# Algy/fast-slic

Hardware: NVIDIA H100
Metric: megapixels/sec (10 iters, K=1600) (higher is better)
Workload: dtype u8/u16 integer

## Files before the change

### fast_slic_b200/csrc/cca.cuh

```cuda
#pragma once
#include "common.cuh"

#define CCA_BLOCK 1024
#define CCA_HIST 2052

struct CcaParams {
    int H, W, N;
    int K;
    int thres;
    int nblk;
    int heap_in_smem;
    int which;
};

__device__ __forceinline__ bool cca_skip_image(const CcaParams& cp, const struct CcaCounters* ct);

struct CcaCounters {
    int ncomp;
    int ncand;
    int nkept;
    int sel_mode;
    int keep_thres;
    int need_sim;
    int dbg_ops;
    int dbg_t;
};

__device__ __forceinline__ bool cca_skip_image(const CcaParams& cp, const CcaCounters* ct) {
    return cp.which >= 0 && (ct->need_sim != 0) != (cp.which != 0);
}

__device__ __forceinline__ int ccl_find(const int* par, int x) {
    int p = par[x];
    while (p != x) {
        x = p;
        p = par[x];
    }
    return x;
}

__device__ __forceinline__ void ccl_union(int* par, int a, int b) {
    a = ccl_find(par, a);
    b = ccl_find(par, b);
    while (a != b) {
        if (a < b) {
            int t = a;
            a = b;
            b = t;
        }
        const int old = atomicMin(&par[a], b);
        if (old == a) break;
        a = ccl_find(par, old);
        b = ccl_find(par, b);
    }
}

#define CCL_T 32

#define CCL_TW 4
__global__ void __launch_bounds__(32 * CCL_TW) k_ccl_tile(CcaParams cp, const uint16_t* __restrict__ labels,
                                                          int* __restrict__ par_all, uint32_t* __restrict__ area_all,
                                                          int tiles_x, int tiles_y, long ntiles_total) {
    __shared__ int s_par_all[CCL_TW][CCL_T * CCL_T];
    const int lane = threadIdx.x & 31, warp = threadIdx.x >> 5;
    const long tile = (long)blockIdx.x * CCL_TW + warp;
    if (tile >= ntiles_total) return;
    int* s_par = s_par_all[warp];
    const int per_img = tiles_x * tiles_y;
    const int b = (int)(tile / per_img);
    const int tl = (int)(tile - (long)b * per_img);
    const int tyb = tl / tiles_x, txb = tl - tyb * tiles_x;
    const int j = txb * CCL_T + lane;
    const bool colok = j < cp.W;
    const int nrows = min(CCL_T, cp.H - tyb * CCL_T);
    const uint16_t* lab = labels + (size_t)b * cp.N + (size_t)(tyb * CCL_T) * cp.W + j;
    constexpr int CCL_G = 8;
    uint32_t v[CCL_G], nv[CCL_G];
#pragma unroll
    for (int k = 0; k < CCL_G; k++) {
        v[k] = (colok && k < nrows) ? (uint32_t)lab[(size_t)k * cp.W] : (0x10000u + (uint32_t)(k * CCL_T + lane));
    }
    uint32_t up_v = 0xffffffffu, up_left = 0xffffffffu;
    int up_root = 0;
#pragma unroll 1
    for (int ty0 = 0; ty0 < CCL_T; ty0 += CCL_G) {
#pragma unroll
        for (int k = 0; k < CCL_G; k++) {
            const int ty = ty0 + CCL_G + k;
            nv[k] = (colok && ty < nrows) ? (uint32_t)lab[(size_t)ty * cp.W] : (0x10000u + (uint32_t)((ty & (CCL_T - 1)) * CCL_T + lane));
        }
#pragma unroll
        for (int k = 0; k < CCL_G; k++) {
            const int ty = ty0 + k;
            const uint32_t cur = v[k];
            const uint32_t left = __shfl_up_sync(FSLIC_FULL, cur, 1);
            const bool start = (lane == 0) || (cur != left);
            const unsigned m = __ballot_sync(FSLIC_FULL, start);
            const int sl = 31 - __clz(m & (0xffffffffu >> (31 - lane)));
            const unsigned above = (lane == 31) ? 0u : (m >> (lane + 1));
            const int end = above ? (lane + __ffs(above) - 1) : 31;
            const bool conn = (ty > 0) && (up_v == cur);
            const bool need = conn && ((lane == 0) || (left != cur) || (up_left != up_v));
            unsigned cand = 0xffffffffu;
            if (need) cand = (unsigned)ccl_find(s_par, up_root);
            unsigned pm = cand;
#pragma unroll
            for (int o = 1; o < 32; o <<= 1) {
                const unsigned y = __shfl_up_sync(FSLIC_FULL, pm, o);
                if (lane - o >= sl) pm = min(pm, y);
            }
            const unsigned rmin = __shfl_sync(FSLIC_FULL, pm, end);
            const unsigned own = (unsigned)(ty * CCL_T + sl);
            const int root = (int)(rmin < own ? rmin : own);
            if (need && cand != (unsigned)root) ccl_union(s_par, (int)cand, root);
            s_par[ty * CCL_T + lane] = root;
            __syncwarp();
            up_left = left;
            up_v = cur;
            up_root = root;
        }
#pragma unroll
        for (int k = 0; k < CCL_G; k++) v[k] = nv[k];
    }
    if (!colok) return;
    int* pout = par_all + (size_t)b * cp.N + (size_t)(tyb * CCL_T) * cp.W + j;
    uint32_t* aout = area_all + (size_t)b * cp.N + (size_t)(tyb * CCL_T) * cp.W + j;
#pragma unroll 4
    for (int ty = 0; ty < nrows; ty++) {
        const int rt = ccl_find(s_par, ty * CCL_T + lane);
        const int ri = tyb * CCL_T + (rt >> 5), rj = txb * CCL_T + (rt & 31);
        pout[(size_t)ty * cp.W] = ri * cp.W + rj;
        aout[(size_t)ty * cp.W] = 0;
    }
}

__global__ void __launch_bounds__(256) k_ccl_seams(CcaParams cp, const uint16_t* __restrict__ labels,
                                                   int* __restrict__ par_all) {
    const int b = blockIdx.y;
    const int W = cp.W, H = cp.H;
    const int sv = (W - 1) / CCL_T, sh = (H - 1) / CCL_T;
    const int nV = sv * H, nH = sh * W;
    const uint16_t* lab = labels + (size_t)b * cp.N;
    int* par = par_all + (size_t)b * cp.N;
    for (int t = blockIdx.x * blockDim.x + threadIdx.x; t < nV + nH; t += gridDim.x * blockDim.x) {
        if (t < nV) {
            const int i = t / sv, j = (t - i * sv + 1) * CCL_T;
            const int p = i * W + j;
            if (lab[p - 1] == lab[p]) ccl_union(par, p - 1, p);
        } else {
            const int u = t - nV;
            const int r = u / W, j = u - r * W;
            const int i = (r + 1) * CCL_T;
            const int p = i * W + j;
            const uint16_t v = lab[p], up = lab[p - W];
            if (up == v) {
                bool need = (j % CCL_T == 0) || (lab[p - 1] != v);
                if (!need) need = lab[p - W - 1] != up;
                if (need) ccl_union(par, p - W, p);
            }
        }
    }
}

__global__ void __launch_bounds__(256) k_ccl_flatten(CcaParams cp, const uint16_t* __restrict__ labels,
                                                     int* __restrict__ par_all, uint32_t* __restrict__ area_all,
                                                     int* __restrict__ blkcnt, int* __restrict__ rootbuf_all,
                                                     int* __restrict__ predbuf_all,
                                                     unsigned long long* __restrict__ chunkinfo_all) {
    __shared__ int s_chunk[32];
    const int b = blockIdx.y;
    const int lane = threadIdx.x & 31, w = threadIdx.x >> 5;
    const uint16_t* lab = labels + (size_t)b * cp.N;
    int* par = par_all + (size_t)b * cp.N;
    int p[4], sl[4], root[4];
    unsigned m[4], rmask[4];
    bool ok[4], start[4], col0[4];
    int jcol = (blockIdx.x * CCA_BLOCK + w * 128 + lane) % cp.W;
#pragma unroll
    for (int r = 0; r < 4; r++) {
        p[r] = blockIdx.x * CCA_BLOCK + (w * 4 + r) * 32 + lane;
        ok[r] = p[r] < cp.N;
        const uint32_t v = ok[r] ? lab[p[r]] : 0x10000u;
        const uint32_t left = __shfl_up_sync(FSLIC_FULL, v, 1);
        const int j = jcol;
        col0[r] = j == 0;
        jcol += 32;
        if (jcol >= cp.W) jcol = (cp.W >= 32) ? (jcol - cp.W) : (jcol % cp.W);
        start[r] = (lane == 0) || (j == 0) || (v != left);
        m[r] = __ballot_sync(FSLIC_FULL, start[r]);
        sl[r] = 31 - __clz(m[r] & (0xffffffffu >> (31 - lane)));
    }
    {
        int q[4];
#pragma unroll
        for (int r = 0; r < 4; r++) {
            root[r] = p[r];
            q[r] = (ok[r] && start[r]) ? par[p[r]] : p[r];
        }
        for (;;) {
            bool mv[4], any = false;
#pragma unroll
            for (int r = 0; r < 4; r++) {
                mv[r] = q[r] != root[r];
                root[r] = q[r];
                any |= mv[r];
            }
            if (!any) break;
#pragma unroll
            for (int r = 0; r < 4; r++)
                if (mv[r]) q[r] = par[root[r]];
        }
    }
    int pred[4], findq[4];
    int prev_last = 0;
#pragma unroll
    for (int r = 0; r < 4; r++) {
        const int rt = __shfl_sync(FSLIC_FULL, root[r], sl[r]);
        const int left_rt = __shfl_up_sync(FSLIC_FULL, rt, 1);
        const int last_rt = __shfl_sync(FSLIC_FULL, rt, 31);
        bool isroot = false;
        pred[r] = -1;
        findq[r] = -1;
        if (ok[r]) {
            par[p[r]] = rt;
            if (start[r]) {
                const unsigned above = (lane == 31) ? 0u : (m[r] >> (lane + 1));
                int len = above ? (__ffs(above)) : (32 - lane);
                if (p[r] + len > cp.N) len = cp.N - p[r];
                atomicAdd(&area_all[(size_t)b * cp.N + rt], (uint32_t)len);
                isroot = (rt == p[r]);
                if (isroot && p[r] > 0) {
                    if (col0[r]) findq[r] = p[r] - cp.W;
                    else if (lane > 0) pred[r] = left_rt;
                    else if (r > 0) pred[r] = prev_last;
                    else findq[r] = p[r] - 1;
                }
            }
        }
        prev_last = last_rt;
        rmask[r] = __ballot_sync(FSLIC_FULL, isroot);
        if (lane == 0) s_chunk[w * 4 + r] = __popc(rmask[r]);
    }
#pragma unroll
    for (int r = 0; r < 4; r++)
        if (findq[r] >= 0) pred[r] = ccl_find(par, findq[r]);
    __syncthreads();
    const int mine = s_chunk[lane];
    int incl = mine;
#pragma unroll
    for (int o = 1; o < 32; o <<= 1) {
        const int y = __shfl_up_sync(FSLIC_FULL, incl, o);
        if (lane >= o) incl += y;
    }
    int* rootbuf = rootbuf_all + (size_t)b * cp.N + (size_t)blockIdx.x * CCA_BLOCK;
    int* predbuf = predbuf_all + (size_t)b * cp.N + (size_t)blockIdx.x * CCA_BLOCK;
#pragma unroll
    for (int r = 0; r < 4; r++) {
        const int base = __shfl_sync(FSLIC_FULL, incl - mine, w * 4 + r);
        if ((rmask[r] >> lane) & 1u) {
            const int e = base + __popc(rmask[r] & ((1u << lane) - 1u));
            rootbuf[e] = p[r];
            predbuf[e] = pred[r];
        }
        if (lane == 0)
            chunkinfo_all[((size_t)b * cp.nblk + blockIdx.x) * (CCA_BLOCK / 32) + w * 4 + r] =
                ((unsigned long long)(unsigned)base << 32) | rmask[r];
    }
    if (threadIdx.x == 31) blkcnt[(size_t)b * cp.nblk + blockIdx.x] = incl;
}

__global__ void __launch_bounds__(1024) k_scan_blocks(const int* __restrict__ cnt_all, int* __restrict__ off_all,
                                                      int stride_per_image, int n_static,
                                                      const int* __restrict__ n_dev_base, int n_dev_stride_ints,
                                                      int n_div, int* __restrict__ total_base,
                                                      int total_stride_ints,
                                                      const CcaCounters* __restrict__ skip_counters, int which) {
    __shared__ int s_warp[32];
    __shared__ int s_carry;
    const int b = blockIdx.x;
    if (skip_counters && which >= 0 && (skip_counters[b].need_sim != 0) != (which != 0)) return;
    const int tid = threadIdx.x;
    const int* cnt = cnt_all + (size_t)b * stride_per_image;
    int* off = off_all + (size_t)b * stride_per_image;
    int n = n_static;
    if (n_dev_base) n = (n_dev_base[(size_t)b * n_dev_stride_ints] + n_div - 1) / n_div;
    if (tid == 0) s_carry = 0;
    __syncthreads();
    for (int base = 0; base < n; base += 1024) {
        const int c = base + tid;
        const int v = (c < n) ? cnt[c] : 0;
        int x = v;
#pragma unroll
        for (int o = 1; o < 32; o <<= 1) {
            int y = __shfl_up_sync(FSLIC_FULL, x, o);
            if ((tid & 31) >= o) x += y;
        }
        if ((tid & 31) == 31) s_warp[tid >> 5] = x;
        __syncthreads();
        if (tid < 32) {
            int w = s_warp[tid];
#pragma unroll
            for (int o = 1; o < 32; o <<= 1) {
                int y = __shfl_up_sync(FSLIC_FULL, w, o);
                if (tid >= o) w += y;
            }
            s_warp[tid] = w;
        }
        __syncthreads();
        const int woff = (tid >> 5) ? s_warp[(tid >> 5) - 1] : 0;
        const int excl = s_carry + woff + x - v;
        if (c < n) off[c] = excl;
        __syncthreads();
        if (tid == 1023) s_carry = excl + v;
        __syncthreads();
    }
    if (tid == 0) total_base[(size_t)b * total_stride_ints] = s_carry;
}

#define CCA_NUMBER_GRID 16
__global__ void __launch_bounds__(CCA_BLOCK) k_ccl_number(CcaParams cp, const int* __restrict__ rootbuf_all,
                                                          const uint32_t* __restrict__ aux_all,
                                                          const int* __restrict__ blkcnt,
                                                          const int* __restrict__ blkoff,
                                                          uint32_t* __restrict__ carea_all,
                                                          CcaCounters* __restrict__ counters,
                                                          unsigned int* __restrict__ ahist_all) {
    __shared__ int s_cand;
    __shared__ unsigned int s_hot[CCA_BLOCK / 32][32];
    const int b = blockIdx.y;
    const int lane = threadIdx.x & 31, warp = threadIdx.x >> 5;
    s_hot[warp][lane] = 0;
    if (threadIdx.x == 0) s_cand = 0;
    __syncthreads();
    const uint32_t* aux = aux_all + (size_t)b * cp.N;
    int ncand = 0;
    constexpr int NU = 8;
    const int wpi = gridDim.x * (CCA_BLOCK / 32);
    const int NB = (cp.nblk + wpi - 1) / wpi;
    for (int blk0 = (blockIdx.x * (CCA_BLOCK / 32) + warp) * NB; blk0 < cp.nblk; blk0 += wpi * NB) {
        for (int sub = 0; sub < NB; sub += 32) {
            const int myblk = blk0 + sub + lane;
            const bool have = (sub + lane < NB) && (myblk < cp.nblk);
            const int mycnt = have ? blkcnt[(size_t)b * cp.nblk + myblk] : 0;
            const int myoff = have ? blkoff[(size_t)b * cp.nblk + myblk] : 0;
            int incl = mycnt;
#pragma unroll
            for (int o = 1; o < 32; o <<= 1) {
                const int y = __shfl_up_sync(FSLIC_FULL, incl, o);
                if (lane >= o) incl += y;
            }
            const int total = __shfl_sync(FSLIC_FULL, incl, 31);
            const int nb_here = min(32, NB - sub);
            for (int r0 = 0; r0 < total; r0 += 32 * NU) {
                int pp[NU], cc[NU];
                uint32_t aa[NU];
#pragma unroll
                for (int u = 0; u < NU; u++) {
                    const int r = r0 + 32 * u + lane;
                    int bi = 0;
                    for (int q = 0; q < nb_here - 1; q++) bi += (r >= __shfl_sync(FSLIC_FULL, incl, q));
                    const int bincl = __shfl_sync(FSLIC_FULL, incl, bi), bcnt = __shfl_sync(FSLIC_FULL, mycnt, bi);
                    const int boff = __shfl_sync(FSLIC_FULL, myoff, bi);
                    const int t = r - (bincl - bcnt);
                    pp[u] = -1;
                    if (r < total) {
                        pp[u] = rootbuf_all[(size_t)b * cp.N + (size_t)(blk0 + sub + bi) * CCA_BLOCK + t];
                        cc[u] = boff + t;
                    }
                }
#pragma unroll
                for (int u = 0; u < NU; u++) aa[u] = pp[u] != -1 ? aux[pp[u]] : 0u;
#pragma unroll
                for (int u = 0; u < NU; u++) {
                    uint32_t bin = 0xffffffffu;
                    if (pp[u] != -1) {
                        carea_all[(size_t)b * cp.N + cc[u]] = aa[u];
                        if ((int)aa[u] >= cp.thres) bin = aa[u] < 2048u ? aa[u] : 2048u;
                    }
                    const unsigned peers = __match_any_sync(FSLIC_FULL, bin);
                    if (bin != 0xffffffffu && lane == __ffs(peers) - 1) {
                        const unsigned n = __popc(peers);
                        ncand += (int)n;
                        if (bin < 32u) s_hot[warp][bin] += n;
                        else atomicAdd(&ahist_all[(size_t)b * CCA_HIST + bin], n);
                    }
                    __syncwarp();
                }
            }
        }
    }
    ncand = __reduce_add_sync(FSLIC_FULL, ncand);
    if (lane == 0 && ncand) atomicAdd(&s_cand, ncand);
    __syncthreads();
    if (threadIdx.x == 0 && s_cand) atomicAdd(&counters[b].ncand, s_cand);
    if (threadIdx.x < 32) {
        unsigned int tot = 0;
        for (int w = 0; w < CCA_BLOCK / 32; w++) tot += s_hot[w][threadIdx.x];
        if (tot) atomicAdd(&ahist_all[(size_t)b * CCA_HIST + threadIdx.x], tot);
    }
}

__global__ void __launch_bounds__(1024) k_cca_threshold(CcaParams cp, const uint32_t* __restrict__ carea_all,
                                                        CcaCounters* __restrict__ counters,
                                                        const unsigned int* __restrict__ ahist_all) {
    __shared__ unsigned int s_hist[2048];
    __shared__ int s_warp[32];
    __shared__ unsigned int s_prefix, s_rank, s_found_bin, s_found_cnt;
    const int b = blockIdx.x;
    const int tid = threadIdx.x, lane = tid & 31, warp = tid >> 5;
    CcaCounters* ct = &counters[b];
    const int ncomp = ct->ncomp, ncand = ct->ncand;
    if (ncand <= cp.K) {
        if (tid == 0) {
            ct->keep_thres = cp.thres;
            ct->sel_mode = 0;
            ct->need_sim = 0;
        }
        return;
    }
    const uint32_t* area = carea_all + (size_t)b * cp.N;
    if (tid == 0) {
// ... 470 lines not shown
    const int b = blockIdx.y;
    if (cca_skip_image(cp, &counters[b])) return;
    const int ncomp = counters[b].ncomp;
    const int sel_mode = counters[b].sel_mode, keep_thres = counters[b].keep_thres;
    const int tid = threadIdx.x, lane = tid & 31, warp = tid >> 5;
    const uint32_t* carea = carea_all + (size_t)b * cp.N;
    for (int blk0 = blockIdx.x * CCA_KEPT_U; blk0 * CCA_BLOCK < ncomp; blk0 += gridDim.x * CCA_KEPT_U) {
        uint32_t a[CCA_KEPT_U];
        int off[CCA_KEPT_U];
#pragma unroll
        for (int u = 0; u < CCA_KEPT_U; u++) {
            const int c = (blk0 + u) * CCA_BLOCK + tid;
            a[u] = (c < ncomp) ? carea[c] : 0u;
            off[u] = ((blk0 + u) * CCA_BLOCK < ncomp) ? blkoff[(size_t)b * cp.nblk + blk0 + u] : 0;
        }
        unsigned m[CCA_KEPT_U];
        bool kept[CCA_KEPT_U];
        __syncthreads();
#pragma unroll
        for (int u = 0; u < CCA_KEPT_U; u++) {
            const int c = (blk0 + u) * CCA_BLOCK + tid;
            kept[u] = (c < ncomp) && cca_is_kept(a[u], sel_mode, keep_thres);
            m[u] = __ballot_sync(FSLIC_FULL, kept[u]);
            if (lane == 0) s_warp[u][warp] = __popc(m[u]);
        }
        __syncthreads();
        if (warp < CCA_KEPT_U) {
            const int w = s_warp[warp][lane];
            int x = w;
#pragma unroll
            for (int o = 1; o < 32; o <<= 1) {
                const int y = __shfl_up_sync(FSLIC_FULL, x, o);
                if (lane >= o) x += y;
            }
            s_warp[warp][lane] = x - w;
        }
        __syncthreads();
#pragma unroll
        for (int u = 0; u < CCA_KEPT_U; u++) {
            const int c = (blk0 + u) * CCA_BLOCK + tid;
            if (c < ncomp) {
                uint16_t v = (c == 0) ? 0 : 0xFFFF;
                if (kept[u]) v = (uint16_t)(off[u] + s_warp[u][warp] + __popc(m[u] & ((1u << lane) - 1)));
                cnew_all[(size_t)b * cp.N + c] = v;
            }
        }
    }
}

#define CCA_TAIL_WARPS 8

__device__ __forceinline__ int cca_comp_of_root(const unsigned long long* chunkinfo, const int* blkoff, int x,
                                                int& slot) {
    const unsigned long long ci = chunkinfo[x >> 5];
    const int local = (int)(ci >> 32) + __popc((uint32_t)ci & ((1u << (x & 31)) - 1u));
    slot = (x >> 10) * CCA_BLOCK + local;
    return blkoff[x >> 10] + local;
}

__device__ __forceinline__ unsigned cca_ld_label(const uint16_t* p) {
    unsigned short v;
    asm volatile("ld.relaxed.gpu.global.u16 %0, [%1];" : "=h"(v) : "l"(p));
    return v;
}
__device__ __forceinline__ void cca_st_label(uint16_t* p, unsigned v) {
    asm volatile("st.relaxed.gpu.global.u16 [%0], %1;" ::"l"(p), "h"((unsigned short)v));
}

__global__ void __launch_bounds__(32 * CCA_TAIL_WARPS) k_cca_absorb(CcaParams cp, const int* __restrict__ rootbuf_all,
                                                                   const int* __restrict__ predbuf_all,
                                                                   const unsigned long long* __restrict__ chunkinfo_all,
                                                                   const int* __restrict__ blkoff_all,
                                                                   const CcaCounters* __restrict__ counters,
                                                                   uint16_t* cnew_all, uint16_t* __restrict__ final_all,
                                                                   int nsplit) {
    const int b = blockIdx.y;
    if (cca_skip_image(cp, &counters[b])) return;
    const int lane = threadIdx.x & 31, gw = blockIdx.x * CCA_TAIL_WARPS + (threadIdx.x >> 5);
    const int blk = gw / nsplit, part = gw - blk * nsplit;
    if (blk >= cp.nblk) return;
    const int* blkoff = blkoff_all + (size_t)b * cp.nblk;
    const int off = blkoff[blk];
    const int n = ((blk + 1 < cp.nblk) ? blkoff[blk + 1] : counters[b].ncomp) - off;
    const int* roots = rootbuf_all + (size_t)b * cp.N + (size_t)blk * CCA_BLOCK;
    const int* preds = predbuf_all + (size_t)b * cp.N;
    const unsigned long long* chunkinfo = chunkinfo_all + (size_t)b * cp.nblk * (CCA_BLOCK / 32);
    uint16_t* cnew = cnew_all + (size_t)b * cp.N;
    uint16_t* fin = final_all + (size_t)b * cp.N;
    constexpr int NU = 8;
    for (int t0 = 32 * part; t0 < n; t0 += 32 * nsplit * NU) {
        int rt[NU], x[NU];
        unsigned lab[NU];
#pragma unroll
        for (int u = 0; u < NU; u++) {
            const int t = t0 + 32 * nsplit * u + lane;
            rt[u] = -1;
            x[u] = 0;
            lab[u] = 0;
            if (t < n) {
                rt[u] = roots[t];
                x[u] = preds[(size_t)blk * CCA_BLOCK + t];
                lab[u] = cnew[off + t];
            }
        }
        int cx[NU], slot[NU];
        unsigned pl[NU];
        bool act[NU];
#pragma unroll
        for (int u = 0; u < NU; u++) {
            act[u] = rt[u] >= 0 && lab[u] == 0xFFFFu;
            pl[u] = 0;
            if (act[u]) cx[u] = cca_comp_of_root(chunkinfo, blkoff, x[u], slot[u]);
        }
        for (;;) {
            bool any = false;
#pragma unroll
            for (int u = 0; u < NU; u++) pl[u] = act[u] ? cca_ld_label(cnew + cx[u]) : pl[u];
#pragma unroll
            for (int u = 0; u < NU; u++) {
                if (act[u] && pl[u] != 0xFFFFu) {
                    act[u] = false;
                    lab[u] = pl[u];
                    cca_st_label(cnew + off + t0 + 32 * nsplit * u + lane, pl[u]);
                }
                any |= act[u];
            }
            if (!any) break;
            int q[NU];
#pragma unroll
            for (int u = 0; u < NU; u++) q[u] = act[u] ? preds[slot[u]] : 0;
#pragma unroll
            for (int u = 0; u < NU; u++)
                if (act[u]) cx[u] = cca_comp_of_root(chunkinfo, blkoff, q[u], slot[u]);
        }
#pragma unroll
        for (int u = 0; u < NU; u++) {
            if (rt[u] < 0) continue;
            fin[rt[u]] = (uint16_t)lab[u];
        }
    }
}

__global__ void __launch_bounds__(256) k_cca_output(CcaParams cp, const int* __restrict__ par_all,
                                                    const uint16_t* __restrict__ final_all,
                                                    uint16_t* __restrict__ out_all,
                                                    const CcaCounters* __restrict__ counters) {
    const int b = blockIdx.y;
    if (cca_skip_image(cp, &counters[b])) return;
    const int* par = par_all + (size_t)b * cp.N;
    const uint16_t* fin = final_all + (size_t)b * cp.N;
    uint16_t* out = out_all + (size_t)b * cp.N;
    if ((cp.N & 7) == 0 && (reinterpret_cast<uintptr_t>(out_all) & 15) == 0 && (reinterpret_cast<uintptr_t>(par_all) & 15) == 0) {
        for (int t = blockIdx.x * blockDim.x + threadIdx.x; t < cp.N / 8; t += gridDim.x * blockDim.x) {
            const int4 r0 = reinterpret_cast<const int4*>(par)[2 * t], r1 = reinterpret_cast<const int4*>(par)[2 * t + 1];
            const uint32_t a0 = fin[r0.x];
            uint32_t a1 = a0, a2, a3, a4, a5, a6, a7;
            if (r0.y != r0.x) a1 = fin[r0.y];
            a2 = a1; if (r0.z != r0.y) a2 = fin[r0.z];
            a3 = a2; if (r0.w != r0.z) a3 = fin[r0.w];
            a4 = a3; if (r1.x != r0.w) a4 = fin[r1.x];
            a5 = a4; if (r1.y != r1.x) a5 = fin[r1.y];
            a6 = a5; if (r1.z != r1.y) a6 = fin[r1.z];
            a7 = a6; if (r1.w != r1.z) a7 = fin[r1.w];
            reinterpret_cast<uint4*>(out)[t] = make_uint4(a0 | (a1 << 16), a2 | (a3 << 16), a4 | (a5 << 16), a6 | (a7 << 16));
        }
        return;
    }
    for (int p = blockIdx.x * blockDim.x + threadIdx.x; p < cp.N; p += gridDim.x * blockDim.x) out[p] = fin[par[p]];
}
```

### fast_slic_b200/csrc/cca_stage.cu

```cuda
#include <stdlib.h>
#include <algorithm>
#include <type_traits>

#include "capi_common.h"
#include "cca.cuh"
#include "cca_stage.h"

struct CcaScratch {
    int* par;
    uint32_t* aux;
    uint32_t* carea;
    uint16_t* cnew;
    uint16_t* fin;
    int* rootbuf;
    int* predbuf;
    unsigned long long* chunkinfo;
    int* blkcnt;
    int* blkoff;
    int* kblkoff;
    CcaCounters* counters;
    unsigned int* ahist;
    unsigned long long* heap;
    size_t total;
};

static CcaScratch cca_layout(void* base, int N, int images, int slot) {
    CcaScratch x;
    Carve c(base);
    auto take = [&](auto*& p, size_t per_image) {
        using T = std::remove_reference_t<decltype(*p)>;
        p = c.take<T>((size_t)images * per_image * sizeof(T));
        if (p) p += (size_t)slot * per_image;
    };
    const size_t n = (size_t)N, nblk = (size_t)ceil_div(N, CCA_BLOCK);
    take(x.par, n);
    take(x.aux, n);
    take(x.carea, n);
    x.cnew = c.take<uint16_t>((size_t)images * n * 2 * sizeof(uint16_t));
    x.fin = x.cnew ? x.cnew + ((size_t)images + slot) * n : nullptr;
    if (x.cnew) x.cnew += (size_t)slot * n;
    take(x.rootbuf, n);
    take(x.predbuf, n);
    take(x.chunkinfo, nblk * (CCA_BLOCK / 32));
    take(x.blkcnt, nblk);
    take(x.blkoff, nblk);
    take(x.kblkoff, nblk);
    take(x.counters, 1);
    take(x.ahist, CCA_HIST);
    take(x.heap, CCA_HEAP_K);
    x.total = c.total;
    return x;
}

static CcaScratch cca_window(const CcaStage& s, int slot) { return cca_layout(s.scratch, s.N, s.batch, slot); }

cudaError_t cca_stage_create(CcaStage& s, int H, int W, int max_batch, size_t device_bytes, int num_sms, int max_smem_optin) {
    s.H = H; s.W = W; s.N = H * W; s.num_sms = num_sms; s.max_smem_optin = max_smem_optin;
    const size_t per_img = (size_t)s.N * 26 + 4096;
    size_t cap = 12ull << 30;
    if (device_bytes && device_bytes / 8 < cap) cap = device_bytes / 8;
    size_t bc = cap / per_img;
    if (bc < 1) bc = 1;
    if (bc > (size_t)max_batch) bc = max_batch;
    if (const char* e = getenv("FSLIC_CCA_BATCH")) {
        const long v = atol(e);
        if (v >= 1 && (size_t)v < bc) bc = (size_t)v;
    }
    s.batch = (int)bc;
    cudaError_t e = cudaMalloc(&s.scratch, cca_layout(nullptr, s.N, s.batch, 0).total);
    if (e == cudaSuccess) e = cudaMemset(cca_window(s, 0).counters, 0, bc * sizeof(CcaCounters));
    if (e == cudaSuccess) e = cudaMallocHost(reinterpret_cast<void**>(&s.h_counters), 64 * sizeof(CcaCounters));
    for (auto& ev : s.ev)
        if (e == cudaSuccess) e = cudaEventCreate(&ev);
    for (CcaLane& l : s.lanes) {
        if (e == cudaSuccess) e = cudaStreamCreateWithFlags(&l.side, cudaStreamNonBlocking);
        for (cudaEvent_t* ev : {&l.fork, &l.join, &l.tail})
            if (e == cudaSuccess) e = cudaEventCreateWithFlags(ev, cudaEventDisableTiming);
    }
    if (e == cudaSuccess)
        e = cudaFuncSetAttribute(k_cca_select, cudaFuncAttributeMaxDynamicSharedMemorySize, max_smem_optin - 4 * 1024);
    if (e == cudaSuccess)
        e = cudaFuncSetAttribute(k_debug_heap_select, cudaFuncAttributeMaxDynamicSharedMemorySize, max_smem_optin - 4 * 1024);
    return e;
}

void cca_stage_destroy(CcaStage& s) {
    if (s.scratch) cudaFree(s.scratch);
    if (s.h_counters) cudaFreeHost(s.h_counters);
    for (cudaEvent_t e : s.ev)
        if (e) cudaEventDestroy(e);
    for (const CcaLane& l : s.lanes) {
        if (l.side) cudaStreamDestroy(l.side);
        for (cudaEvent_t e : {l.fork, l.join, l.tail})
            if (e) cudaEventDestroy(e);
    }
}

static int number_grid(int nblk, int nb) {
    return nb >= 8 ? CCA_NUMBER_GRID : std::min(std::max(ceil_div(nblk, 32), CCA_NUMBER_GRID), 64);
}

static int cca_label(const CcaStage& s, const CcaScratch& x, const CcaParams& cp, const uint16_t* in, int nb, bool timed,
                     cudaStream_t st) {
    if (timed) CK(cudaEventRecord(s.ev[0], st));
    CK(cudaMemsetAsync(x.counters, 0, sizeof(CcaCounters) * nb, st));
    CK(cudaMemsetAsync(x.ahist, 0, sizeof(unsigned int) * CCA_HIST * nb, st));
    dim3 g(cp.nblk, nb);
    {
        const int ttx = ceil_div(s.W, CCL_T), tty = ceil_div(s.H, CCL_T);
        const long ntt = (long)ttx * tty * nb;
        k_ccl_tile<<<(int)((ntt + CCL_TW - 1) / CCL_TW), 32 * CCL_TW, 0, st>>>(cp, in, x.par, x.aux, ttx, tty, ntt);
    }
    {
        const int seam_px = ((s.W - 1) / CCL_T) * s.H + ((s.H - 1) / CCL_T) * s.W;
        if (seam_px > 0) {
            dim3 gs(ceil_div(seam_px, 256), nb);
            k_ccl_seams<<<gs, 256, 0, st>>>(cp, in, x.par);
        }
    }
    if (timed) CK(cudaEventRecord(s.ev[1], st));
    k_ccl_flatten<<<g, 256, 0, st>>>(cp, in, x.par, x.aux, x.blkcnt, x.rootbuf, x.predbuf, x.chunkinfo);
    k_scan_blocks<<<nb, 1024, 0, st>>>(x.blkcnt, x.blkoff, cp.nblk, cp.nblk, nullptr, 0, 1,
                                       &x.counters[0].ncomp, (int)(sizeof(CcaCounters) / sizeof(int)), nullptr, -1);
    k_ccl_number<<<dim3(number_grid(cp.nblk, nb), nb), CCA_BLOCK, 0, st>>>(cp, x.rootbuf, x.aux, x.blkcnt, x.blkoff,
                                                                            x.carea, x.counters, x.ahist);
    if (timed) CK(cudaEventRecord(s.ev[2], st));
    k_cca_threshold<<<nb, 1024, 0, st>>>(cp, x.carea, x.counters, x.ahist);
    if (timed) CK(cudaEventRecord(s.ev[3], st));
    return FSLIC_OK;
}

static void cca_finish(const CcaStage& s, const CcaScratch& x, const CcaParams& cp, int which, uint16_t* out, int nb,
                       bool timed, cudaStream_t ts) {
    CcaParams cq = cp;
    cq.which = which;
    const dim3 gk(std::min(cp.nblk, std::max(CCA_KEPT_GRID, 256 / nb)), nb);
    k_kept_count<<<gk, CCA_BLOCK, 0, ts>>>(cq, x.carea, x.counters, x.blkcnt);
    k_scan_blocks<<<nb, 1024, 0, ts>>>(x.blkcnt, x.kblkoff, cp.nblk, 0, &x.counters[0].ncomp,
                                       (int)(sizeof(CcaCounters) / sizeof(int)), CCA_BLOCK,
                                       &x.counters[0].nkept, (int)(sizeof(CcaCounters) / sizeof(int)),
                                       x.counters, which);
    k_kept_label<<<gk, CCA_BLOCK, 0, ts>>>(cq, x.carea, x.counters, x.kblkoff, x.cnew);
    if (timed) cudaEventRecord(s.ev[4], ts);
    const int nsplit = nb < 4 ? 8 : 1;
    const dim3 ga(ceil_div(cp.nblk * nsplit, CCA_TAIL_WARPS), nb);
    k_cca_absorb<<<ga, 32 * CCA_TAIL_WARPS, 0, ts>>>(cq, x.rootbuf, x.predbuf, x.chunkinfo, x.blkoff, x.counters,
                                                      x.cnew, x.fin, nsplit);
    if (timed) cudaEventRecord(s.ev[5], ts);
    int ob = ceil_div(ceil_div(s.N, 8), 256);
    if (ob > s.num_sms * 32) ob = s.num_sms * 32;
    dim3 go(ob, nb);
    k_cca_output<<<go, 256, 0, ts>>>(cq, x.par, x.fin, out, x.counters);
    if (timed) cudaEventRecord(s.ev[6], ts);
}

static int cca_copy_runs(const CcaCounters* hcnt, int nb, bool replayed, const uint16_t* out, size_t N, const HostOut& ho) {
    int b = 0;
    while (b < nb) {
        if ((hcnt[b].need_sim != 0) != replayed) { b++; continue; }
        int e = b;
        while (e < nb && (hcnt[e].need_sim != 0) == replayed) e++;
        CK(cudaMemcpyAsync(ho.h_labels + (size_t)b * N, out + (size_t)b * N, (size_t)(e - b) * N * 2,
                           cudaMemcpyDeviceToHost, ho.out_stream));
        b = e;
    }
    return FSLIC_OK;
}

int cca_run(CcaStage& s, CcaDispatch& d, const uint16_t* d_in, uint16_t* d_out, int batch, int K, int thres,
            cudaStream_t st, int* launches, HostOut* ho, int slot, int lane) {
    const int N = s.N;
    if (slot != 0 && slot + batch > s.batch) return set_err(FSLIC_EINVAL, "scratch window out of range");
    const CcaScratch x = cca_window(s, slot);
    CcaCounters* const hcnt = s.h_counters + slot;
    const CcaLane& ln = s.lanes[lane];
    CcaParams cp;
    cp.H = s.H; cp.W = s.W; cp.N = N; cp.K = K; cp.thres = thres; cp.which = -1;
    cp.nblk = ceil_div(N, CCA_BLOCK);
    const size_t heap_bytes = (size_t)(2 * K + 4) * 8;
    cp.heap_in_smem = heap_bytes + SEL_CHUNK * 8 <= (size_t)(s.max_smem_optin - 8 * 1024);
    if (K + 2 > CCA_HEAP_K) return set_err(FSLIC_EINVAL, "K too large for the selection heap");
    d.heap_smem = cp.heap_in_smem ? 1 : 0;
    d.heap_smem_max_k =
        (int)std::max<long>(0, ((long)s.max_smem_optin - 8 * 1024 - SEL_CHUNK * 8) / 8 / 2 - 2);
    d.sub_batches = ceil_div(batch, s.batch);
    for (int b0 = 0; b0 < batch; b0 += s.batch) {
        const int nb = (batch - b0 < s.batch) ? (batch - b0) : s.batch;
        const uint16_t* in = d_in + (size_t)b0 * N;
        uint16_t* out = d_out + (size_t)b0 * N;
        const bool timed = s.timing && nb < 4 && batch <= s.batch;
        s.timed = timed;
        int rc = cca_label(s, x, cp, in, nb, timed, st);
        if (rc) return rc;
        if (b0 == 0) {
            d.split = nb >= 4;
            d.number_nb = ceil_div(cp.nblk, number_grid(cp.nblk, nb) * (CCA_BLOCK / 32));
        }
        const bool split = nb >= 4;
        const bool early = split && ho && batch <= s.batch && nb <= 64;
        if (early) {
            CK(cudaMemcpyAsync(hcnt, x.counters, sizeof(CcaCounters) * nb, cudaMemcpyDeviceToHost, st));
            CK(cudaStreamSynchronize(st));
        }
        if (split) {
            CK(cudaEventRecord(ln.fork, st));
            CK(cudaStreamWaitEvent(ln.side, ln.fork, 0));
            cca_finish(s, x, cp, 0, out, nb, timed, ln.side);
            CK(cudaEventRecord(ln.join, ln.side));
        }
        if (early) {
            CK(cudaStreamWaitEvent(ho->out_stream, ln.join, 0));
            rc = cca_copy_runs(hcnt, nb, false, out, N, *ho);
            if (rc) return rc;
        }
        k_cca_select<<<nb, 1024, SEL_CHUNK * 8 + (cp.heap_in_smem ? heap_bytes : 0), st>>>(cp, x.carea, x.counters, x.heap);
        cca_finish(s, x, cp, split ? 1 : -1, out, nb, timed, st);
        if (early) {
            CK(cudaEventRecord(ln.tail, st));
            CK(cudaStreamWaitEvent(ho->out_stream, ln.tail, 0));
            rc = cca_copy_runs(hcnt, nb, true, out, N, *ho);
            if (rc) return rc;
            ho->done = true;
        }
        if (split) {
            CK(cudaStreamWaitEvent(st, ln.join, 0));
            if (launches) *launches += 5;
        }
        CK(cudaGetLastError());
        if (launches) *launches += 12;
    }
    return FSLIC_OK;
}

void cca_set_timing(CcaStage& s, bool on) {
    s.timing = on;
    s.timed = false;
}

void cca_read_timing(CcaStage& s) {
    for (int i = 0; i < 6; i++) {
        float ms;
        s.ms[i] = 0.f;
        if (s.timed && cudaEventElapsedTime(&ms, s.ev[i], s.ev[i + 1]) == cudaSuccess) s.ms[i] = ms;
    }
    cudaGetLastError();
}

void cca_sync_lanes(const CcaStage& s) {
    for (const CcaLane& l : s.lanes)
        if (l.side) cudaStreamSynchronize(l.side);
}

int cca_heap_select(const CcaStage& s, const int32_t* d_area, int n, int middle, uint8_t* d_kept, cudaStream_t st) {
    CK(cudaMemsetAsync(d_kept, 0, n, st));
    const size_t hb = (size_t)(2 * middle + 4) * 8;
    const int use_smem = hb + SEL_CHUNK * 8 <= (size_t)(s.max_smem_optin - 8 * 1024);
    k_debug_heap_select<<<1, 1024, SEL_CHUNK * 8 + (use_smem ? hb : 0), st>>>(reinterpret_cast<const uint32_t*>(d_area), n,
                                                                              middle, d_kept, cca_window(s, 0).heap, use_smem);
    CK(cudaGetLastError());
    return FSLIC_OK;
}

int cca_read_counters(const CcaStage& s, int32_t* out8, int image) {
    CK(cudaDeviceSynchronize());
    CK(cudaMemcpy(out8, cca_window(s, image).counters, sizeof(CcaCounters), cudaMemcpyDeviceToHost));
    return FSLIC_OK;
}

void cca_read_dispatch(const CcaDispatch& d, int32_t* out, int count) {
    const int32_t v[FSLIC_CCA_DISPATCH_COUNT] = {d.heap_smem, d.heap_smem_max_k, d.sub_batches, d.split, d.number_nb};
    for (int i = 0; i < count && i < FSLIC_CCA_DISPATCH_COUNT; i++) out[i] = v[i];
}

void cca_read_ms(const CcaStage& s, float* out_ms, int count) {
    for (int i = 0; i < count && i < 6; i++) out_ms[i] = s.ms[i];
}
```

Measured before the change: 16270.

## Compute tile-local areas and closed roots in tile kernel, resolve only open components

The tile CCL kernel now accumulates per-root run lengths in shared memory and marks components that touch tile borders as open. Closed roots are recorded directly in chunkinfo, and only open roots are listed for a new k_ccl_open kernel that merges their areas into global roots. The full-image flatten pass is replaced by a lighter k_ccl_roots pass that builds root and predecessor buffers from the chunk masks. Because par is no longer fully flattened, later lookups do an extra indirection. This adds memsets, a launch, and correctness risk around the pred lookup, which now assumes at most two hops.

```diff
diff --git a/fast_slic_b200/csrc/cca.cuh b/fast_slic_b200/csrc/cca.cuh
--- a/fast_slic_b200/csrc/cca.cuh
+++ b/fast_slic_b200/csrc/cca.cuh
@@ -58,14 +58,22 @@
 #define CCL_T 32
 
 #define CCL_TW 4
+#define CCL_OPEN 0x8000u
+
 __global__ void __launch_bounds__(32 * CCL_TW) k_ccl_tile(CcaParams cp, const uint16_t* __restrict__ labels,
-                                                          int* __restrict__ par_all, uint32_t* __restrict__ area_all,
+                                                          int* __restrict__ par_all, uint32_t* __restrict__ aux_all,
+                                                          unsigned long long* __restrict__ chunkinfo_all,
+                                                          int* __restrict__ open_all, int* __restrict__ nopen,
                                                           int tiles_x, int tiles_y, long ntiles_total) {
     __shared__ int s_par_all[CCL_TW][CCL_T * CCL_T];
+    __shared__ unsigned s_rec_all[CCL_TW][CCL_T * CCL_T / 2];
     const int lane = threadIdx.x & 31, warp = threadIdx.x >> 5;
     const long tile = (long)blockIdx.x * CCL_TW + warp;
     if (tile >= ntiles_total) return;
     int* s_par = s_par_all[warp];
+    unsigned* s_rec = s_rec_all[warp];
+#pragma unroll
+    for (int k = 0; k < CCL_T / 2; k++) s_rec[k * CCL_T + lane] = 0;
     const int per_img = tiles_x * tiles_y;
     const int b = (int)(tile / per_img);
     const int tl = (int)(tile - (long)b * per_img);
@@ -74,6 +82,19 @@
     const bool colok = j < cp.W;
     const int nrows = min(CCL_T, cp.H - tyb * CCL_T);
     const uint16_t* lab = labels + (size_t)b * cp.N + (size_t)(tyb * CCL_T) * cp.W + j;
+    unsigned contacts;
+    {
+        const uint16_t* row = labels + (size_t)b * cp.N + (size_t)(tyb * CCL_T + lane) * cp.W + txb * CCL_T;
+        const int last = min(CCL_T, cp.W - txb * CCL_T) - 1;
+        const bool rok = lane < nrows;
+        const bool lc = rok && txb > 0 && row[-1] == row[0];
+        const bool rc = rok && last == CCL_T - 1 && txb * CCL_T + CCL_T < cp.W && row[CCL_T] == row[CCL_T - 1];
+        const unsigned lm = __ballot_sync(FSLIC_FULL, lc), rm = __ballot_sync(FSLIC_FULL, rc);
+        contacts = (lane == 0) ? lm : (lane == 31) ? rm : 0u;
+    }
+    const uint32_t above_v = (colok && tyb > 0) ? (uint32_t)lab[-(ptrdiff_t)cp.W] : 0xffffffffu;
+    const uint32_t below_v = (colok && nrows == CCL_T && (tyb + 1) * CCL_T < cp.H) ? (uint32_t)lab[(size_t)CCL_T * cp.W]
+                                                                                  : 0xffffffffu;
     constexpr int CCL_G = 8;
     uint32_t v[CCL_G], nv[CCL_G];
 #pragma unroll
@@ -82,6 +103,7 @@
     }
     uint32_t up_v = 0xffffffffu, up_left = 0xffffffffu;
     int up_root = 0;
+    unsigned run_starts = 0;
 #pragma unroll 1
     for (int ty0 = 0; ty0 < CCL_T; ty0 += CCL_G) {
 #pragma unroll
@@ -96,6 +118,9 @@
             const uint32_t left = __shfl_up_sync(FSLIC_FULL, cur, 1);
             const bool start = (lane == 0) || (cur != left);
             const unsigned m = __ballot_sync(FSLIC_FULL, start);
+            if (lane == ty) run_starts = m;
+            const bool vcontact = (ty == 0 && above_v == cur) || (ty == CCL_T - 1 && below_v == cur);
+            contacts |= (unsigned)vcontact << ty;
             const int sl = 31 - __clz(m & (0xffffffffu >> (31 - lane)));
             const unsigned above = (lane == 31) ? 0u : (m >> (lane + 1));
             const int end = above ? (lane + __ffs(above) - 1) : 31;
@@ -122,15 +147,59 @@
 #pragma unroll
         for (int k = 0; k < CCL_G; k++) v[k] = nv[k];
     }
-    if (!colok) return;
-    int* pout = par_all + (size_t)b * cp.N + (size_t)(tyb * CCL_T) * cp.W + j;
-    uint32_t* aout = area_all + (size_t)b * cp.N + (size_t)(tyb * CCL_T) * cp.W + j;
+    const int row0 = tyb * CCL_T;
+    int* pout = par_all + (size_t)b * cp.N + (size_t)row0 * cp.W + j;
 #pragma unroll 4
     for (int ty = 0; ty < nrows; ty++) {
         const int rt = ccl_find(s_par, ty * CCL_T + lane);
-        const int ri = tyb * CCL_T + (rt >> 5), rj = txb * CCL_T + (rt & 31);
-        pout[(size_t)ty * cp.W] = ri * cp.W + rj;
-        aout[(size_t)ty * cp.W] = 0;
+        const unsigned m = __shfl_sync(FSLIC_FULL, run_starts, ty);
+        if (colok) {
+            const int sh = (rt & 1) * 16;
+            if ((m >> lane) & 1u) {
+                const unsigned above = (lane == 31) ? 0u : (m >> (lane + 1));
+                atomicAdd(&s_rec[rt >> 1], (above ? __ffs(above) : 32 - lane) << sh);
+            }
+            if ((contacts >> ty) & 1u) atomicOr(&s_rec[rt >> 1], CCL_OPEN << sh);
+            pout[(size_t)ty * cp.W] = (row0 + (rt >> 5)) * cp.W + txb * CCL_T + (rt & 31);
+        }
+    }
+    __syncwarp();
+    uint32_t* aux = aux_all + (size_t)b * cp.N;
+    unsigned long long* chunkinfo = chunkinfo_all + (size_t)b * cp.nblk * (CCA_BLOCK / 32);
+    unsigned open_rows = 0;
+    for (int ty = 0; ty < nrows; ty++) {
+        const int x = ty * CCL_T + lane;
+        const bool isroot = colok && s_par[x] == x;
+        const unsigned rec = (s_rec[x >> 1] >> ((x & 1) * 16)) & 0xffffu;
+        const int g = (row0 + ty) * cp.W + j;
+        if (isroot) aux[g] = rec & (CCL_OPEN - 1);
+        const unsigned closed = __ballot_sync(FSLIC_FULL, isroot && !(rec & CCL_OPEN));
+        const unsigned opened = __ballot_sync(FSLIC_FULL, isroot && (rec & CCL_OPEN));
+        if (lane == ty) open_rows = opened;
+        if (lane == 0 && closed) {
+            const int s = g & 31;
+            atomicOr(&chunkinfo[g >> 5], (unsigned long long)(closed << s));
+            if (s && (closed >> (32 - s))) atomicOr(&chunkinfo[(g >> 5) + 1], (unsigned long long)(closed >> (32 - s)));
+        }
+    }
+    const int cnt = __popc(open_rows);
+    int incl = cnt;
+#pragma unroll
+    for (int o = 1; o < 32; o <<= 1) {
+        const int y = __shfl_up_sync(FSLIC_FULL, incl, o);
+        if (lane >= o) incl += y;
+    }
+    const int total = __shfl_sync(FSLIC_FULL, incl, 31);
+    if (total == 0) return;
+    int base = 0;
+    if (lane == 0) base = atomicAdd(&nopen[b], total);
+    base = __shfl_sync(FSLIC_FULL, base, 0);
+    int* open_list = open_all + (size_t)b * cp.N;
+    for (unsigned rows = __ballot_sync(FSLIC_FULL, cnt != 0); rows; rows &= rows - 1) {
+        const int ty = __ffs(rows) - 1;
+        const unsigned om = __shfl_sync(FSLIC_FULL, open_rows, ty);
+        const int e = base + __shfl_sync(FSLIC_FULL, incl - cnt, ty) + __popc(om & ((1u << lane) - 1u));
+        if ((om >> lane) & 1u) open_list[e] = (row0 + ty) * cp.W + j;
     }
 }
 
@@ -162,111 +231,82 @@
     }
 }
 
-__global__ void __launch_bounds__(256) k_ccl_flatten(CcaParams cp, const uint16_t* __restrict__ labels,
-                                                     int* __restrict__ par_all, uint32_t* __restrict__ area_all,
-                                                     int* __restrict__ blkcnt, int* __restrict__ rootbuf_all,
-                                                     int* __restrict__ predbuf_all,
-                                                     unsigned long long* __restrict__ chunkinfo_all) {
-    __shared__ int s_chunk[32];
+__global__ void __launch_bounds__(256) k_ccl_open(CcaParams cp, int* __restrict__ par_all, uint32_t* __restrict__ aux_all,
+                                                  unsigned long long* __restrict__ chunkinfo_all,
+                                                  const int* __restrict__ open_all, const int* __restrict__ nopen) {
     const int b = blockIdx.y;
-    const int lane = threadIdx.x & 31, w = threadIdx.x >> 5;
-    const uint16_t* lab = labels + (size_t)b * cp.N;
+    const int n = nopen[b];
     int* par = par_all + (size_t)b * cp.N;
-    int p[4], sl[4], root[4];
-    unsigned m[4], rmask[4];
-    bool ok[4], start[4], col0[4];
-    int jcol = (blockIdx.x * CCA_BLOCK + w * 128 + lane) % cp.W;
-#pragma unroll
-    for (int r = 0; r < 4; r++) {
-        p[r] = blockIdx.x * CCA_BLOCK + (w * 4 + r) * 32 + lane;
-        ok[r] = p[r] < cp.N;
-        const uint32_t v = ok[r] ? lab[p[r]] : 0x10000u;
-        const uint32_t left = __shfl_up_sync(FSLIC_FULL, v, 1);
-        const int j = jcol;
-        col0[r] = j == 0;
-        jcol += 32;
-        if (jcol >= cp.W) jcol = (cp.W >= 32) ? (jcol - cp.W) : (jcol % cp.W);
-        start[r] = (lane == 0) || (j == 0) || (v != left);
-        m[r] = __ballot_sync(FSLIC_FULL, start[r]);
-        sl[r] = 31 - __clz(m[r] & (0xffffffffu >> (31 - lane)));
-    }
-    {
-        int q[4];
-#pragma unroll
-        for (int r = 0; r < 4; r++) {
-            root[r] = p[r];
-            q[r] = (ok[r] && start[r]) ? par[p[r]] : p[r];
-        }
-        for (;;) {
-            bool mv[4], any = false;
-#pragma unroll
-            for (int r = 0; r < 4; r++) {
-                mv[r] = q[r] != root[r];
-                root[r] = q[r];
-                any |= mv[r];
-            }
-            if (!any) break;
-#pragma unroll
-            for (int r = 0; r < 4; r++)
-                if (mv[r]) q[r] = par[root[r]];
-        }
-    }
-    int pred[4], findq[4];
-    int prev_last = 0;
-#pragma unroll
-    for (int r = 0; r < 4; r++) {
-        const int rt = __shfl_sync(FSLIC_FULL, root[r], sl[r]);
-        const int left_rt = __shfl_up_sync(FSLIC_FULL, rt, 1);
-        const int last_rt = __shfl_sync(FSLIC_FULL, rt, 31);
-        bool isroot = false;
-        pred[r] = -1;
-        findq[r] = -1;
-        if (ok[r]) {
-            par[p[r]] = rt;
-            if (start[r]) {
-                const unsigned above = (lane == 31) ? 0u : (m[r] >> (lane + 1));
-                int len = above ? (__ffs(above)) : (32 - lane);
-                if (p[r] + len > cp.N) len = cp.N - p[r];
-                atomicAdd(&area_all[(size_t)b * cp.N + rt], (uint32_t)len);
-                isroot = (rt == p[r]);
-                if (isroot && p[r] > 0) {
-                    if (col0[r]) findq[r] = p[r] - cp.W;
-                    else if (lane > 0) pred[r] = left_rt;
-                    else if (r > 0) pred[r] = prev_last;
-                    else findq[r] = p[r] - 1;
-                }
-            }
-        }
-        prev_last = last_rt;
-        rmask[r] = __ballot_sync(FSLIC_FULL, isroot);
-        if (lane == 0) s_chunk[w * 4 + r] = __popc(rmask[r]);
-    }
-#pragma unroll
-    for (int r = 0; r < 4; r++)
-        if (findq[r] >= 0) pred[r] = ccl_find(par, findq[r]);
-    __syncthreads();
-    const int mine = s_chunk[lane];
-    int incl = mine;
+    uint32_t* aux = aux_all + (size_t)b * cp.N;
+    unsigned long long* chunkinfo = chunkinfo_all + (size_t)b * cp.nblk * (CCA_BLOCK / 32);
+    const int* open_list = open_all + (size_t)b * cp.N;
+    for (int i = blockIdx.x * blockDim.x + threadIdx.x; i < n; i += gridDim.x * blockDim.x) {
+        const int t = open_list[i];
+        const int g = ccl_find(par, t);
+        if (g != t) {
+            par[t] = g;
+            atomicAdd(&aux[g], aux[t]);
+        } else {
+            atomicOr(&chunkinfo[g >> 5], 1ull << (g & 31));
+        }
+    }
+}
+
+#define CCL_ROOTS_WARPS 8
+__global__ void __launch_bounds__(32 * CCL_ROOTS_WARPS) k_ccl_roots(CcaParams cp, const int* __restrict__ par_all,
+                                                                    int* __restrict__ blkcnt,
+                                                                    int* __restrict__ rootbuf_all,
+                                                                    int* __restrict__ predbuf_all,
+                                                                    unsigned long long* __restrict__ chunkinfo_all) {
+    const int b = blockIdx.y;
+    const int lane = threadIdx.x & 31;
+    const int blk = blockIdx.x * CCL_ROOTS_WARPS + (threadIdx.x >> 5);
+    if (blk >= cp.nblk) return;
+    const int* par = par_all + (size_t)b * cp.N;
+    unsigned long long* ci = chunkinfo_all + ((size_t)b * cp.nblk + blk) * (CCA_BLOCK / 32) + lane;
+    const uint32_t mask = (uint32_t)*ci;
+    const int cnt = __popc(mask);
+    int incl = cnt;
 #pragma unroll
     for (int o = 1; o < 32; o <<= 1) {
         const int y = __shfl_up_sync(FSLIC_FULL, incl, o);
         if (lane >= o) incl += y;
     }
-    int* rootbuf = rootbuf_all + (size_t)b * cp.N + (size_t)blockIdx.x * CCA_BLOCK;
-    int* predbuf = predbuf_all + (size_t)b * cp.N + (size_t)blockIdx.x * CCA_BLOCK;
-#pragma unroll
-    for (int r = 0; r < 4; r++) {
-        const int base = __shfl_sync(FSLIC_FULL, incl - mine, w * 4 + r);
-        if ((rmask[r] >> lane) & 1u) {
-            const int e = base + __popc(rmask[r] & ((1u << lane) - 1u));
-            rootbuf[e] = p[r];
-            predbuf[e] = pred[r];
-        }
-        if (lane == 0)
-            chunkinfo_all[((size_t)b * cp.nblk + blockIdx.x) * (CCA_BLOCK / 32) + w * 4 + r] =
-                ((unsigned long long)(unsigned)base << 32) | rmask[r];
-    }
-    if (threadIdx.x == 31) blkcnt[(size_t)b * cp.nblk + blockIdx.x] = incl;
+    *ci = ((unsigned long long)(unsigned)(incl - cnt) << 32) | mask;
+    if (lane == 31) blkcnt[(size_t)b * cp.nblk + blk] = incl;
+    int* rootbuf = rootbuf_all + (size_t)b * cp.N + (size_t)blk * CCA_BLOCK;
+    int* predbuf = predbuf_all + (size_t)b * cp.N + (size_t)blk * CCA_BLOCK;
+    const int p0 = blk * CCA_BLOCK + lane;
+    int jcol = p0 % cp.W;
+    constexpr int CCL_RU = 8;
+#pragma unroll 1
+    for (int c0 = 0; c0 < CCA_BLOCK / 32; c0 += CCL_RU) {
+        uint32_t m[CCL_RU];
+        int q[CCL_RU];
+#pragma unroll
+        for (int u = 0; u < CCL_RU; u++) {
+            m[u] = __shfl_sync(FSLIC_FULL, mask, c0 + u);
+            const int p = p0 + (c0 + u) * 32;
+            q[u] = -1;
+            if (((m[u] >> lane) & 1u) && p > 0) q[u] = jcol == 0 ? p - cp.W : p - 1;
+            jcol += 32;
+            if (jcol >= cp.W) jcol = (cp.W >= 32) ? (jcol - cp.W) : (jcol % cp.W);
+        }
+#pragma unroll
+        for (int u = 0; u < CCL_RU; u++)
+            if (q[u] >= 0) q[u] = par[q[u]];
+#pragma unroll
+        for (int u = 0; u < CCL_RU; u++)
+            if (q[u] >= 0) q[u] = par[q[u]];
+#pragma unroll
+        for (int u = 0; u < CCL_RU; u++) {
+            const int e = __shfl_sync(FSLIC_FULL, incl - cnt, c0 + u) + __popc(m[u] & ((1u << lane) - 1u));
+            if ((m[u] >> lane) & 1u) {
+                rootbuf[e] = p0 + (c0 + u) * 32;
+                predbuf[e] = q[u];
+            }
+        }
+    }
 }
 
 __global__ void __launch_bounds__(1024) k_scan_blocks(const int* __restrict__ cnt_all, int* __restrict__ off_all,
@@ -1043,7 +1083,16 @@
     uint16_t* out = out_all + (size_t)b * cp.N;
     if ((cp.N & 7) == 0 && (reinterpret_cast<uintptr_t>(out_all) & 15) == 0 && (reinterpret_cast<uintptr_t>(par_all) & 15) == 0) {
         for (int t = blockIdx.x * blockDim.x + threadIdx.x; t < cp.N / 8; t += gridDim.x * blockDim.x) {
-            const int4 r0 = reinterpret_cast<const int4*>(par)[2 * t], r1 = reinterpret_cast<const int4*>(par)[2 * t + 1];
+            const int4 t0 = reinterpret_cast<const int4*>(par)[2 * t], t1 = reinterpret_cast<const int4*>(par)[2 * t + 1];
+            int4 r0, r1;
+            r0.x = par[t0.x];
+            r0.y = r0.x; if (t0.y != t0.x) r0.y = par[t0.y];
+            r0.z = r0.y; if (t0.z != t0.y) r0.z = par[t0.z];
+            r0.w = r0.z; if (t0.w != t0.z) r0.w = par[t0.w];
+            r1.x = r0.w; if (t1.x != t0.w) r1.x = par[t1.x];
+            r1.y = r1.x; if (t1.y != t1.x) r1.y = par[t1.y];
+            r1.z = r1.y; if (t1.z != t1.y) r1.z = par[t1.z];
+            r1.w = r1.z; if (t1.w != t1.z) r1.w = par[t1.w];
             const uint32_t a0 = fin[r0.x];
             uint32_t a1 = a0, a2, a3, a4, a5, a6, a7;
             if (r0.y != r0.x) a1 = fin[r0.y];
@@ -1057,5 +1106,5 @@
         }
         return;
     }
-    for (int p = blockIdx.x * blockDim.x + threadIdx.x; p < cp.N; p += gridDim.x * blockDim.x) out[p] = fin[par[p]];
-}
+    for (int p = blockIdx.x * blockDim.x + threadIdx.x; p < cp.N; p += gridDim.x * blockDim.x) out[p] = fin[par[par[p]]];
+}
diff --git a/fast_slic_b200/csrc/cca_stage.cu b/fast_slic_b200/csrc/cca_stage.cu
--- a/fast_slic_b200/csrc/cca_stage.cu
+++ b/fast_slic_b200/csrc/cca_stage.cu
@@ -15,6 +15,7 @@
     int* rootbuf;
     int* predbuf;
     unsigned long long* chunkinfo;
+    int* nopen;
     int* blkcnt;
     int* blkoff;
     int* kblkoff;
@@ -42,6 +43,7 @@
     take(x.rootbuf, n);
     take(x.predbuf, n);
     take(x.chunkinfo, nblk * (CCA_BLOCK / 32));
+    take(x.nopen, 1);
     take(x.blkcnt, nblk);
     take(x.blkoff, nblk);
     take(x.kblkoff, nblk);
@@ -105,11 +107,13 @@
     if (timed) CK(cudaEventRecord(s.ev[0], st));
     CK(cudaMemsetAsync(x.counters, 0, sizeof(CcaCounters) * nb, st));
     CK(cudaMemsetAsync(x.ahist, 0, sizeof(unsigned int) * CCA_HIST * nb, st));
-    dim3 g(cp.nblk, nb);
+    CK(cudaMemsetAsync(x.chunkinfo, 0, sizeof(unsigned long long) * cp.nblk * (CCA_BLOCK / 32) * nb, st));
+    CK(cudaMemsetAsync(x.nopen, 0, sizeof(int) * nb, st));
+    const int ttx = ceil_div(s.W, CCL_T), tty = ceil_div(s.H, CCL_T);
     {
-        const int ttx = ceil_div(s.W, CCL_T), tty = ceil_div(s.H, CCL_T);
         const long ntt = (long)ttx * tty * nb;
-        k_ccl_tile<<<(int)((ntt + CCL_TW - 1) / CCL_TW), 32 * CCL_TW, 0, st>>>(cp, in, x.par, x.aux, ttx, tty, ntt);
+        k_ccl_tile<<<(int)((ntt + CCL_TW - 1) / CCL_TW), 32 * CCL_TW, 0, st>>>(cp, in, x.par, x.aux, x.chunkinfo,
+                                                                               x.predbuf, x.nopen, ttx, tty, ntt);
     }
     {
         const int seam_px = ((s.W - 1) / CCL_T) * s.H + ((s.H - 1) / CCL_T) * s.W;
@@ -119,7 +123,9 @@
         }
     }
     if (timed) CK(cudaEventRecord(s.ev[1], st));
-    k_ccl_flatten<<<g, 256, 0, st>>>(cp, in, x.par, x.aux, x.blkcnt, x.rootbuf, x.predbuf, x.chunkinfo);
+    k_ccl_open<<<dim3(ceil_div(ttx * tty * 32, 256), nb), 256, 0, st>>>(cp, x.par, x.aux, x.chunkinfo, x.predbuf, x.nopen);
+    k_ccl_roots<<<dim3(ceil_div(cp.nblk, CCL_ROOTS_WARPS), nb), 32 * CCL_ROOTS_WARPS, 0, st>>>(cp, x.par, x.blkcnt, x.rootbuf,
+                                                                                              x.predbuf, x.chunkinfo);
     k_scan_blocks<<<nb, 1024, 0, st>>>(x.blkcnt, x.blkoff, cp.nblk, cp.nblk, nullptr, 0, 1,
                                        &x.counters[0].ncomp, (int)(sizeof(CcaCounters) / sizeof(int)), nullptr, -1);
     k_ccl_number<<<dim3(number_grid(cp.nblk, nb), nb), CCA_BLOCK, 0, st>>>(cp, x.rootbuf, x.aux, x.blkcnt, x.blkoff,
@@ -227,7 +233,7 @@
             if (launches) *launches += 5;
         }
         CK(cudaGetLastError());
-        if (launches) *launches += 12;
+        if (launches) *launches += 13;
     }
     return FSLIC_OK;
 }
```

New measurement: 15860, median of 6. -2.5%, worse.
